# anshium/visual-place-recognition-and-geopose-estimation

Hardware: AMD Instinct MI355X
Metric: images/sec end-to-end (backbone->SALAD->kNN->pose) (higher is better)
Workload: dtype bf16; 1 GPU; DINOv2 vit_large/14 (random init) + SALAD + bf16 kNN k=10 over a 100000-row x 8448 synthetic gallery sharded 1 way(s) + fused (lat,lon,sin,cos) head; 3x224x224 bf16 images; batch_per_gpu=64, global_batch=64, gallery_rows=100000, k=10, parallelism=dp1+gallery-shard1, batches_in_flight=1, graph_retrieval=False

## Files before the change

visual-place-recognition-and-geopose-estimation_amd/csrc/attention.hip:

```cpp
#include <stdlib.h>
#include "vpr_common.h"
#include "vpr_internal.h"

namespace vpr {

constexpr int AT_D = 64;
constexpr int AT_KP = 288;


__device__ __forceinline__ int vtile_off(int row, int chunk) { return row * 128 + ((chunk ^ (row & 7)) << 4); }

struct AttnCtx {
  const char* Ks; const char* Vs; const uint16_t* qb; long long tok_stride; int T, qcol, g, trq, trp;
  float scale_log2e; uint16_t* out; long long out_stride;
  long long row_base, tail_base; int Tp;
};
__device__ __forceinline__ long long attn_row(const AttnCtx& cx, int t) {
  return t < cx.Tp ? cx.row_base + t : cx.tail_base + (t - cx.Tp);
}
typedef __attribute__((ext_vector_type(4))) short s16x4;

__device__ __forceinline__ void attn_load_q(const AttnCtx& cx, int qt, bf16x8 (&bq)[2]) {
  const int qrow = min(qt * 16 + cx.qcol, cx.T - 1);
#pragma unroll
  for (int s = 0; s < 2; ++s)
    bq[s] = *reinterpret_cast<const bf16x8*>(cx.qb + attn_row(cx, qrow) * cx.tok_stride + 32 * s + 8 * cx.g);
}
__device__ __forceinline__ f32x4 attn_qk_block(const AttnCtx& cx, int kb, const bf16x8 (&bq)[2]) {
  f32x4 acc = {0.f, 0.f, 0.f, 0.f};
#pragma unroll
  for (int s = 0; s < 2; ++s)
    acc = __builtin_amdgcn_mfma_f32_16x16x32_bf16(lds_frag(cx.Ks, 16 * kb + cx.qcol, cx.g + 4 * s), bq[s], acc, 0, 0, 0);
  return acc;
}
__device__ __forceinline__ void attn_qk_all(const AttnCtx& cx, const bf16x8 (&bq)[2], f32x4 (&sc)[AT_KP / 16]) {
#pragma unroll
  for (int kb = 0; kb < AT_KP / 16; ++kb) {
    sc[kb] = attn_qk_block(cx, kb, bq);
    if ((kb % 3) == 2) __builtin_amdgcn_sched_barrier(0);
  }
}
__device__ __forceinline__ void attn_mask_block(f32x4& s, int kb, int klast, int lim) {
  if (kb > klast) {
    asm volatile("");
    s = f32x4{-INFINITY, -INFINITY, -INFINITY, -INFINITY};
  } else if (kb == klast) {
    asm volatile("");
#pragma unroll
    for (int e = 0; e < 4; ++e) s[e] = e < lim ? s[e] : -INFINITY;
  }
}
__device__ __forceinline__ float attn_rowmax(const AttnCtx& cx, f32x4 (&sc)[AT_KP / 16]) {
  const int klast = (cx.T - 1) >> 4;
  const int lim = cx.T - 16 * klast - 4 * cx.g;
  if (klast < AT_KP / 16 - 2) {
#pragma unroll
    for (int kb = 0; kb < AT_KP / 16 - 2; ++kb) attn_mask_block(sc[kb], kb, klast, lim);
  }
#pragma unroll
  for (int kb = AT_KP / 16 - 2; kb < AT_KP / 16; ++kb) attn_mask_block(sc[kb], kb, klast, lim);
  float mx = sc[0][0];
#pragma unroll
  for (int kb = 0; kb < AT_KP / 16; ++kb) {
    mx = fmaxf(fmaxf(mx, sc[kb][0]), sc[kb][1]);
    mx = fmaxf(fmaxf(mx, sc[kb][2]), sc[kb][3]);
  }
  mx = fmaxf(mx, __shfl_xor(mx, 16, 64));
  return fmaxf(mx, __shfl_xor(mx, 32, 64));
}
__device__ __forceinline__ void attn_phase1(const AttnCtx& cx, f32x4 (&sc)[AT_KP / 16], float mx,
                                             bf16x8 (&pb)[AT_KP / 32], bool has_next, const bf16x8 (&bq)[2]) {
  const float nm = -mx * cx.scale_log2e;
#pragma unroll
  for (int t = 0; t < AT_KP / 32; ++t) {
    float p[8];
#pragma unroll
    for (int e = 0; e < 4; ++e) {
      p[e] = __builtin_amdgcn_exp2f(fmaf(sc[2 * t][e], cx.scale_log2e, nm));
      p[4 + e] = __builtin_amdgcn_exp2f(fmaf(sc[2 * t + 1][e], cx.scale_log2e, nm));
    }
    if (has_next) {
      sc[2 * t] = attn_qk_block(cx, 2 * t, bq);
      sc[2 * t + 1] = attn_qk_block(cx, 2 * t + 1, bq);
    }
#pragma unroll
    for (int j = 0; j < 8; ++j) pb[t][j] = (__bf16)p[j];
  }
}
__device__ __forceinline__ float attn_phase2(const AttnCtx& cx, const bf16x8 (&pb)[AT_KP / 32], int qt, bool has_next, f32x4 (&sn)[AT_KP / 16]) {
  const bf16x8 ones = {(__bf16)1.f, (__bf16)1.f, (__bf16)1.f, (__bf16)1.f, (__bf16)1.f, (__bf16)1.f, (__bf16)1.f, (__bf16)1.f};
  f32x4 sacc = {0.f, 0.f, 0.f, 0.f};
#pragma unroll
  for (int t = 0; t < AT_KP / 32; ++t) sacc = __builtin_amdgcn_mfma_f32_16x16x32_bf16(ones, pb[t], sacc, 0, 0, 0);
  f32x4 oacc[4];
#pragma unroll
  for (int db = 0; db < 4; ++db) {
    oacc[db] = f32x4{0.f, 0.f, 0.f, 0.f};
#pragma unroll
    for (int t = 0; t < AT_KP / 32; ++t) {
      const int r0 = 32 * t + 4 * cx.g + cx.trq;
      const s16x4 lo = __builtin_amdgcn_ds_read_tr16_b64_v4i16(
          (__attribute__((address_space(3))) s16x4*)(cx.Vs + vtile_off(r0, 2 * db + (cx.trp >> 1)) + 8 * (cx.trp & 1)));
      const s16x4 hi = __builtin_amdgcn_ds_read_tr16_b64_v4i16(
          (__attribute__((address_space(3))) s16x4*)(cx.Vs + vtile_off(r0 + 16, 2 * db + (cx.trp >> 1)) + 8 * (cx.trp & 1)));
      const s16x8 av = {lo[0], lo[1], lo[2], lo[3], hi[0], hi[1], hi[2], hi[3]};
      oacc[db] = __builtin_amdgcn_mfma_f32_16x16x32_bf16(__builtin_bit_cast(bf16x8, av), pb[t], oacc[db], 0, 0, 0);
      if ((t % 3) == 2) __builtin_amdgcn_sched_barrier(0);
    }
  }
  const float inv = 1.0f / sacc[0];
  float mxn = 0.f;
  if (has_next) mxn = attn_rowmax(cx, sn);
  const int q = qt * 16 + cx.qcol;
  if (q < cx.T) {
    uint16_t* orow = cx.out + attn_row(cx, q) * cx.out_stride;
#pragma unroll
    for (int db = 0; db < 4; ++db) {
      ushort4 o;
      o.x = f32_to_bf16_bits(oacc[db][0] * inv);
      o.y = f32_to_bf16_bits(oacc[db][1] * inv);
      o.z = f32_to_bf16_bits(oacc[db][2] * inv);
      o.w = f32_to_bf16_bits(oacc[db][3] * inv);
      *reinterpret_cast<ushort4*>(orow + 16 * db + 4 * cx.g) = o;
    }
  }
  return mxn;
}

template <int NW, bool PIPE, int ABL = 0>
__global__ __launch_bounds__(NW * 64, NW / 2) void attention_kernel(
    const uint16_t* __restrict__ qkv, uint16_t* __restrict__ out, int T, int Tp, long long tail_row0, int H,
    float scale_log2e, int dephase) {
  extern __shared__ __attribute__((aligned(16))) char smem[];
  if (dephase > 0 && blockIdx.x >= 256 && blockIdx.x < 512)
    for (int i = 0; i < dephase; ++i) __builtin_amdgcn_s_sleep(33);
  char* Ks = smem;
  char* Vs = smem + AT_KP * 128;
  const int bh = blockIdx.x, b = bh / H, h = bh % H;
  const int tid = threadIdx.x, lane = tid & 63, wave = tid >> 6;
  const long long tok_stride = 3LL * H * AT_D;
  const uint16_t* qb = qkv + (long long)h * AT_D;
  const uint16_t* kb_ = qb + (long long)H * AT_D;
  const uint16_t* vb = qb + 2LL * H * AT_D;

  constexpr int NT = NW * 64;
  constexpr int AT_MAXT = (AT_KP / 16 + NW - 1) / NW;
  bf16x8 qf[AT_MAXT][2];
  {
    AttnCtx c0;
    c0.qb = qb; c0.tok_stride = tok_stride; c0.T = T; c0.qcol = lane & 15; c0.g = lane >> 4;
    c0.Tp = Tp; c0.row_base = (long long)b * Tp; c0.tail_base = tail_row0 + (long long)b * (T - Tp);
#pragma unroll
    for (int j = 0; j < AT_MAXT; ++j) attn_load_q(c0, min(wave + NW * j, ((T + 15) >> 4) - 1), qf[j]);
  }
  constexpr int NLD = (AT_KP * 8 + NT - 1) / NT;
  s16x8 kreg[NLD], vreg[NLD];
#pragma unroll
  for (int it = 0; it < NLD; ++it) {
    const int i = min(tid + NT * it, AT_KP * 8 - 1);
    const int key = i >> 3, ch = i & 7;
    const int kc = key < T ? key : T - 1;
    const long long krow = kc < Tp ? (long long)b * Tp + kc : tail_row0 + (long long)b * (T - Tp) + (kc - Tp);
    kreg[it] = *reinterpret_cast<const s16x8*>(kb_ + krow * tok_stride + ch * 8);
    vreg[it] = *reinterpret_cast<const s16x8*>(vb + krow * tok_stride + ch * 8);
  }
#pragma unroll
  for (int it = 0; it < NLD; ++it) {
    const int i = min(tid + NT * it, AT_KP * 8 - 1);
    const int key = i >> 3, ch = i & 7;
    const s16x8 z = {0, 0, 0, 0, 0, 0, 0, 0};
    const s16x8 kv = key < T ? kreg[it] : z, vv = key < T ? vreg[it] : z;
    *reinterpret_cast<s16x8*>(Ks + tile_off(key, ch)) = kv;
    *reinterpret_cast<s16x8*>(Vs + vtile_off(key, ch)) = vv;
  }
  __syncthreads();

  if (ABL == 3) return;
  const int qcol = lane & 15, g = lane >> 4;
  const int ntile = (T + 15) >> 4;

  AttnCtx cx;
  cx.Ks = Ks; cx.Vs = Vs; cx.qb = qb; cx.tok_stride = tok_stride; cx.T = T; cx.qcol = qcol; cx.g = g;
  cx.trq = (lane & 15) >> 2; cx.trp = lane & 3; cx.scale_log2e = scale_log2e;
  cx.out = out + (long long)h * AT_D; cx.out_stride = (long long)H * AT_D;
  cx.Tp = Tp; cx.row_base = (long long)b * Tp; cx.tail_base = tail_row0 + (long long)b * (T - Tp);

  f32x4 sc[AT_KP / 16];
  bf16x8 pb[AT_KP / 32];
  if (wave >= ntile) return;
  if constexpr (PIPE) {
    attn_qk_all(cx, qf[0], sc);
    float mx = attn_rowmax(cx, sc);
#pragma unroll
    for (int j = 0; j < AT_MAXT; ++j) {
      const int qt = wave + NW * j;
      if (qt < ntile) {
        const bool has_next = qt + NW < ntile;
        attn_phase1(cx, sc, mx, pb, has_next, qf[j + 1 < AT_MAXT ? j + 1 : j]);
        mx = attn_phase2(cx, pb, qt, has_next, sc);
      }
    }
  } else {
#pragma unroll
    for (int j = 0; j < AT_MAXT; ++j) {
      const int qt = wave + NW * j;
      if (qt < ntile) {
        attn_qk_all(cx, qf[j], sc);
        if (ABL == 4) {
          float a = 0.f;
#pragma unroll
          for (int kb = 0; kb < AT_KP / 16; ++kb) a += sc[kb][0] + sc[kb][1] + sc[kb][2] + sc[kb][3];
          if (qt * 16 + cx.qcol < T) cx.out[attn_row(cx, qt * 16 + cx.qcol) * cx.out_stride + 4 * cx.g] = f32_to_bf16_bits(a);
          continue;
        }
        const float mx = attn_rowmax(cx, sc);
        attn_phase1(cx, sc, mx, pb, false, qf[j]);
        if (ABL == 2) {
          float a = 0.f;
#pragma unroll
          for (int t = 0; t < AT_KP / 32; ++t)
#pragma unroll
            for (int e = 0; e < 8; ++e) a += (float)pb[t][e];
          if (qt * 16 + cx.qcol < T) cx.out[attn_row(cx, qt * 16 + cx.qcol) * cx.out_stride + 4 * cx.g] = f32_to_bf16_bits(a);
          continue;
        }
        attn_phase2(cx, pb, qt, false, sc);
      }
    }
  }
}

constexpr size_t AT_LDS = (size_t)2 * AT_KP * 128;

}

using namespace vpr;

static int attention_launch(const uint16_t* qkv, uint16_t* out, int B, int T, int Tp, long long tail_row0, int H,
                            int head_dim, float scale, void* stream) {
  if (!qkv || !out || B <= 0 || T <= 0 || H <= 0 || Tp < 0 || Tp > T || tail_row0 < 0) return VPR_ERR_INVALID_ARG;
  if (!(scale > 0.f && scale <= 3.4e38f)) return VPR_ERR_INVALID_ARG;
  if (head_dim != AT_D || T > AT_KP || (long long)B * H > 0x7fffffffLL) return VPR_ERR_UNSUPPORTED;
  if ((reinterpret_cast<uintptr_t>(qkv) | reinterpret_cast<uintptr_t>(out)) & 15) return VPR_ERR_UNSUPPORTED;
  const int variant = tune_or(TUNE_ATTN_VARIANT, 0);
  const float c = scale * 1.4426950408889634f;
  const int dephase = (variant >= 20 && variant <= 60) ? variant - 20 : 0;
  hipStream_t st = static_cast<hipStream_t>(stream);
#define VPR_ATTN_LAUNCH(NW, PIPE)                                                                        \
  do {                                                                                                   \
    VPR_TRY_LAUNCH((launch_kernel_lds<attention_kernel<NW, PIPE>>(dim3((unsigned)(B * H)), dim3(NW * 64), AT_LDS, st, \
                                                                  qkv, out, T, Tp, tail_row0, H, c, dephase)));     \
  } while (0)
#ifdef VPR_ABLATION
#define VPR_ATTN_ABL(A)                                                                                   \
  do {                                                                                                   \
    VPR_TRY_LAUNCH((launch_kernel_lds<attention_kernel<8, false, A>>(dim3((unsigned)(B * H)), dim3(512), AT_LDS, st, \
                                                                     qkv, out, T, Tp, tail_row0, H, c, 0)));        \
  } while (0)
#endif
  switch (variant) {
    case 1: VPR_ATTN_LAUNCH(4, false); break;
    case 2: VPR_ATTN_LAUNCH(4, true); break;
    case 3: VPR_ATTN_LAUNCH(6, false); break;
#ifdef VPR_ABLATION
    case 12: VPR_ATTN_ABL(2); break;
    case 13: VPR_ATTN_ABL(3); break;
    case 14: VPR_ATTN_ABL(4); break;
#endif
    default: VPR_ATTN_LAUNCH(8, false); break;
  }
#undef VPR_ATTN_LAUNCH
#ifdef VPR_ABLATION
#undef VPR_ATTN_ABL
#endif
  return VPR_OK;
}

extern "C" int vpr_attention_qkv_bf16(const uint16_t* qkv, uint16_t* out, int B, int T, int H, int head_dim,
                                      float scale, void* stream) {
  return attention_launch(qkv, out, B, T, T, 0, H, head_dim, scale, stream);
}

extern "C" int vpr_attention_qkv_split_bf16(const uint16_t* qkv, uint16_t* out, int B, int T, int body_tokens,
                                            long long tail_row0, int H, int head_dim, float scale, void* stream) {
  return attention_launch(qkv, out, B, T, body_tokens, tail_row0, H, head_dim, scale, stream);
}
```

Baseline: 5588 images/s.

## Split K/V staging by wave role and overlap first QK with V stores

The default 8-wave attention kernel now splits the K/V staging between waves: the first half of the waves load K and the second half load V. K is written to LDS and synchronized first, so the K-role waves can compute their first QK tile while the V-role waves write V to LDS, followed by a second barrier. This aims to hide the V staging latency behind the first score computation and to halve the per-thread register staging. It adds an extra __syncthreads, and the dephase window now uses the real CU count instead of a hard-coded 256.

```diff
diff --git a/visual-place-recognition-and-geopose-estimation_amd/csrc/attention.hip b/visual-place-recognition-and-geopose-estimation_amd/csrc/attention.hip
--- a/visual-place-recognition-and-geopose-estimation_amd/csrc/attention.hip
+++ b/visual-place-recognition-and-geopose-estimation_amd/csrc/attention.hip
@@ -127,17 +127,19 @@
   return mxn;
 }
 
-template <int NW, bool PIPE, int ABL = 0>
+template <int NW, bool PIPE, int ABL = 0, bool SPLIT = false>
 __global__ __launch_bounds__(NW * 64, NW / 2) void attention_kernel(
     const uint16_t* __restrict__ qkv, uint16_t* __restrict__ out, int T, int Tp, long long tail_row0, int H,
-    float scale_log2e, int dephase) {
+    float scale_log2e, int dephase, int ncu) {
+  static_assert(!SPLIT || (NW == 8 && !PIPE && ABL == 0), "role-split staging is the 8-wave default's");
   extern __shared__ __attribute__((aligned(16))) char smem[];
-  if (dephase > 0 && blockIdx.x >= 256 && blockIdx.x < 512)
+  if (dephase > 0 && blockIdx.x >= (unsigned)ncu && blockIdx.x < 2u * (unsigned)ncu)
     for (int i = 0; i < dephase; ++i) __builtin_amdgcn_s_sleep(33);
   char* Ks = smem;
   char* Vs = smem + AT_KP * 128;
   const int bh = blockIdx.x, b = bh / H, h = bh % H;
-  const int tid = threadIdx.x, lane = tid & 63, wave = tid >> 6;
+  const int tid = threadIdx.x, lane = tid & 63;
+  const int wave = SPLIT ? __builtin_amdgcn_readfirstlane(tid >> 6) : tid >> 6;
   const long long tok_stride = 3LL * H * AT_D;
   const uint16_t* qb = qkv + (long long)h * AT_D;
   const uint16_t* kb_ = qb + (long long)H * AT_D;
@@ -153,40 +155,73 @@
 #pragma unroll
     for (int j = 0; j < AT_MAXT; ++j) attn_load_q(c0, min(wave + NW * j, ((T + 15) >> 4) - 1), qf[j]);
   }
-  constexpr int NLD = (AT_KP * 8 + NT - 1) / NT;
-  s16x8 kreg[NLD], vreg[NLD];
-#pragma unroll
-  for (int it = 0; it < NLD; ++it) {
-    const int i = min(tid + NT * it, AT_KP * 8 - 1);
-    const int key = i >> 3, ch = i & 7;
-    const int kc = key < T ? key : T - 1;
-    const long long krow = kc < Tp ? (long long)b * Tp + kc : tail_row0 + (long long)b * (T - Tp) + (kc - Tp);
-    kreg[it] = *reinterpret_cast<const s16x8*>(kb_ + krow * tok_stride + ch * 8);
-    vreg[it] = *reinterpret_cast<const s16x8*>(vb + krow * tok_stride + ch * 8);
-  }
-#pragma unroll
-  for (int it = 0; it < NLD; ++it) {
-    const int i = min(tid + NT * it, AT_KP * 8 - 1);
-    const int key = i >> 3, ch = i & 7;
-    const s16x8 z = {0, 0, 0, 0, 0, 0, 0, 0};
-    const s16x8 kv = key < T ? kreg[it] : z, vv = key < T ? vreg[it] : z;
-    *reinterpret_cast<s16x8*>(Ks + tile_off(key, ch)) = kv;
-    *reinterpret_cast<s16x8*>(Vs + vtile_off(key, ch)) = vv;
-  }
-  __syncthreads();
-
-  if (ABL == 3) return;
   const int qcol = lane & 15, g = lane >> 4;
   const int ntile = (T + 15) >> 4;
-
   AttnCtx cx;
   cx.Ks = Ks; cx.Vs = Vs; cx.qb = qb; cx.tok_stride = tok_stride; cx.T = T; cx.qcol = qcol; cx.g = g;
   cx.trq = (lane & 15) >> 2; cx.trp = lane & 3; cx.scale_log2e = scale_log2e;
   cx.out = out + (long long)h * AT_D; cx.out_stride = (long long)H * AT_D;
   cx.Tp = Tp; cx.row_base = (long long)b * Tp; cx.tail_base = tail_row0 + (long long)b * (T - Tp);
-
   f32x4 sc[AT_KP / 16];
   bf16x8 pb[AT_KP / 32];
+
+  bool krole = false;
+  if constexpr (SPLIT) {
+    constexpr int NH = NT / 2, NLD = AT_KP * 8 / NH;
+    static_assert(NLD * NH == AT_KP * 8, "each half covers its matrix exactly");
+    krole = wave < NW / 2;
+    const uint16_t* src = krole ? kb_ : vb;
+    const int t2 = tid & (NH - 1);
+    s16x8 reg[NLD];
+#pragma unroll
+    for (int it = 0; it < NLD; ++it) {
+      const int i = t2 + NH * it, key = i >> 3, ch = i & 7;
+      reg[it] = s16x8{0, 0, 0, 0, 0, 0, 0, 0};
+      if (key < T) reg[it] = *reinterpret_cast<const s16x8*>(src + attn_row(cx, key) * tok_stride + ch * 8);
+    }
+    if (krole) {
+#pragma unroll
+      for (int it = 0; it < NLD; ++it) {
+        const int i = t2 + NH * it;
+        *reinterpret_cast<s16x8*>(Ks + tile_off(i >> 3, i & 7)) = reg[it];
+      }
+    }
+    __syncthreads();
+    if (krole) {
+      if (wave < ntile) attn_qk_all(cx, qf[0], sc);
+    } else {
+#pragma unroll
+      for (int it = 0; it < NLD; ++it) {
+        const int i = t2 + NH * it;
+        *reinterpret_cast<s16x8*>(Vs + vtile_off(i >> 3, i & 7)) = reg[it];
+      }
+    }
+    __syncthreads();
+  } else {
+    constexpr int NLD = (AT_KP * 8 + NT - 1) / NT;
+    s16x8 kreg[NLD], vreg[NLD];
+#pragma unroll
+    for (int it = 0; it < NLD; ++it) {
+      const int i = min(tid + NT * it, AT_KP * 8 - 1);
+      const int key = i >> 3, ch = i & 7;
+      const int kc = key < T ? key : T - 1;
+      const long long krow = kc < Tp ? (long long)b * Tp + kc : tail_row0 + (long long)b * (T - Tp) + (kc - Tp);
+      kreg[it] = *reinterpret_cast<const s16x8*>(kb_ + krow * tok_stride + ch * 8);
+      vreg[it] = *reinterpret_cast<const s16x8*>(vb + krow * tok_stride + ch * 8);
+    }
+#pragma unroll
+    for (int it = 0; it < NLD; ++it) {
+      const int i = min(tid + NT * it, AT_KP * 8 - 1);
+      const int key = i >> 3, ch = i & 7;
+      const s16x8 z = {0, 0, 0, 0, 0, 0, 0, 0};
+      const s16x8 kv = key < T ? kreg[it] : z, vv = key < T ? vreg[it] : z;
+      *reinterpret_cast<s16x8*>(Ks + tile_off(key, ch)) = kv;
+      *reinterpret_cast<s16x8*>(Vs + vtile_off(key, ch)) = vv;
+    }
+    __syncthreads();
+  }
+
+  if (ABL == 3) return;
   if (wave >= ntile) return;
   if constexpr (PIPE) {
     attn_qk_all(cx, qf[0], sc);
@@ -205,7 +240,7 @@
     for (int j = 0; j < AT_MAXT; ++j) {
       const int qt = wave + NW * j;
       if (qt < ntile) {
-        attn_qk_all(cx, qf[j], sc);
+        if (!(SPLIT && j == 0 && krole)) attn_qk_all(cx, qf[j], sc);
         if (ABL == 4) {
           float a = 0.f;
 #pragma unroll
@@ -245,29 +280,31 @@
   const int variant = tune_or(TUNE_ATTN_VARIANT, 0);
   const float c = scale * 1.4426950408889634f;
   const int dephase = (variant >= 20 && variant <= 60) ? variant - 20 : 0;
+  const int ncu = dephase > 0 ? device_cu_count() : 0;
   hipStream_t st = static_cast<hipStream_t>(stream);
-#define VPR_ATTN_LAUNCH(NW, PIPE)                                                                        \
+#define VPR_ATTN_LAUNCH(NW, PIPE, SPLIT)                                                                \
   do {                                                                                                   \
-    VPR_TRY_LAUNCH((launch_kernel_lds<attention_kernel<NW, PIPE>>(dim3((unsigned)(B * H)), dim3(NW * 64), AT_LDS, st, \
-                                                                  qkv, out, T, Tp, tail_row0, H, c, dephase)));     \
+    VPR_TRY_LAUNCH((launch_kernel_lds<attention_kernel<NW, PIPE, 0, SPLIT>>(dim3((unsigned)(B * H)), dim3(NW * 64), AT_LDS, st, \
+                                                                            qkv, out, T, Tp, tail_row0, H, c, dephase, ncu))); \
   } while (0)
 #ifdef VPR_ABLATION
 #define VPR_ATTN_ABL(A)                                                                                   \
   do {                                                                                                   \
     VPR_TRY_LAUNCH((launch_kernel_lds<attention_kernel<8, false, A>>(dim3((unsigned)(B * H)), dim3(512), AT_LDS, st, \
-                                                                     qkv, out, T, Tp, tail_row0, H, c, 0)));        \
+                                                                     qkv, out, T, Tp, tail_row0, H, c, 0, 0)));     \
   } while (0)
 #endif
   switch (variant) {
-    case 1: VPR_ATTN_LAUNCH(4, false); break;
-    case 2: VPR_ATTN_LAUNCH(4, true); break;
-    case 3: VPR_ATTN_LAUNCH(6, false); break;
+    case 1: VPR_ATTN_LAUNCH(4, false, false); break;
+    case 2: VPR_ATTN_LAUNCH(4, true, false); break;
+    case 3: VPR_ATTN_LAUNCH(6, false, false); break;
+    case 5: VPR_ATTN_LAUNCH(8, false, false); break;
 #ifdef VPR_ABLATION
     case 12: VPR_ATTN_ABL(2); break;
     case 13: VPR_ATTN_ABL(3); break;
     case 14: VPR_ATTN_ABL(4); break;
 #endif
-    default: VPR_ATTN_LAUNCH(8, false); break;
+    default: VPR_ATTN_LAUNCH(8, false, true); break;
   }
 #undef VPR_ATTN_LAUNCH
 #ifdef VPR_ABLATION
```

After: 5585 images/s. About the same (-0.0%).
